# phantomzone-org/fhe-ram

Measured on AMD Instinct MI355X. Metric: encrypted RAM read ops/s + write ops/s at 2^18 entries; achieved HBM GB/s vs peak, higher is better.
Workload: dtype f64

## Files before the change

fhe-ram_amd/csrc/launch.hpp:

```cpp
#pragma once
#include "ctx.hpp"

namespace {

template <typename F>
void with_evk(const fheram_ctx* c, F&& f) {
    if (c->s_evk == 5) f(std::integral_constant<int, 5>{});
    else f(std::integral_constant<int, 4>{});
}
template <typename F>
void with_evk_wide(fheram_ctx* c, bool wide, F&& f) {
    if (wide) c->wide_unsynced = true;
    with_evk(c, [&](auto sk) { if (wide) f(sk, std::true_type{}); else f(sk, std::false_type{}); });
}
bool capturing(const fheram_ctx* c) { return c->use_graph && !c->profile; }

constexpr int LIMB_SPLIT_MAX = 64;
constexpr int EW_SLICES = 8;
int pick_nco(const fheram_ctx* c, int gx, int gy, bool one_wg = false) {
    if (c->nco != 0) return c->nco;
    if (one_wg) return 2;
    return ((long)gx * gy * 2 <= c->cus) ? 1 : 2;
}
void launch_prepare(fheram_ctx* c, const int32_t* in, double* out, int npoly, int64_t gal = 0) {
    ProfScope ps(c, "prepare", npoly);
    const int ginv = gal == 0 ? 0 : galois_inv_mod(galois_mod(gal));
    hipLaunchKernelGGL(k_prepare, dim3((npoly + 1) / 2), dim3(T), LDS_PREPARE_BYTES, c->cur, in, out, c->d_tw, c->ninv, ginv, npoly);
}
double* big_of(const fheram_ctx* c) { return c->cur == c->stream2 ? c->d_big2 : c->d_big; }
bool use_limb_split(const fheram_ctx* c, int gx, int gy, int sk) {
    return c->limb_split && (long)gx * gy <= LIMB_SPLIT_MAX && (long)gx * gy * 2 * sk <= c->cus;
}
bool use_fine_split(const fheram_ctx* c, int gx, int gy, int wgs) {
    return c->limb_split && c->fine_split && (long)gx * gy * wgs <= c->cus && (long)gx * gy * wgs * N * 8 <= (long)LIMB_SPLIT_MAX * BIG_STRIDE * 8;
}
void launch_ep(fheram_ctx* c, GlweRef a, GlweRef res, const double* ggsw, int gx, int gy) {
    if (gx <= 0 || gy <= 0) return;
    ProfScope ps(c, "ext_product", (uint64_t)gx * gy);
    if (use_fine_split(c, gx, gy, 2 * 4 * 2 * 3)) {
        hipLaunchKernelGGL((k_ext_product_fine<3, 4>), dim3(gx, gy, 2 * 4 * 2 * 3), dim3(T), LDS_BYTES, c->cur, a, ggsw, c->d_tw, big_of(c));
        hipLaunchKernelGGL((k_ext_product_fine_norm<3, 4>), dim3(gx, gy, 2 * (N / 256)), dim3(256), 0, c->cur, res, big_of(c));
        return;
    }
    if (use_limb_split(c, gx, gy, 4)) {
        hipLaunchKernelGGL((k_ext_product<3, 4, 1, 1>), dim3(gx, gy, 8), dim3(T), LDS_BYTES, c->cur, a, res, ggsw, c->d_tw, big_of(c));
        hipLaunchKernelGGL((k_ext_product<3, 4, 1, 2>), dim3(gx, gy, 2), dim3(T), 0, c->cur, a, res, ggsw, c->d_tw, big_of(c));
        return;
    }
    if (pick_nco(c, gx, gy) == 1) hipLaunchKernelGGL((k_ext_product<3, 4, 1>), dim3(gx, gy, 2), dim3(T), LDS_BYTES, c->cur, a, res, ggsw, c->d_tw, big_of(c));
    else {
        ProfScope pf(c, "ext_product_fused", (uint64_t)gx * gy);
        hipLaunchKernelGGL((k_ext_product<3, 4, 2>), dim3(gx, gy, 1), dim3(T), LDS_BYTES, c->cur, a, res, ggsw, c->d_tw, big_of(c));
    }
}
template <int MODE, int SX, int SK, int SO>
void launch_ks(fheram_ctx* c, const KsArgs& ka, int gx, int gy) {
    if (gx <= 0 || gy <= 0) return;
    ProfScope ps(c, "keyswitch", (uint64_t)gx * gy);
    if (use_fine_split(c, gx, gy, 2 * SK * SX)) {
        KsArgs kb = ka;
        kb.big = big_of(c);
        hipLaunchKernelGGL((k_keyswitch_fine<MODE, SX, SK>), dim3(gx, gy, 2 * SK * SX), dim3(T), LDS_BYTES, c->cur, kb);
        hipLaunchKernelGGL((k_keyswitch_norm<MODE, SX, SK, SO, SX>), dim3(gx, gy, 2 * (N / 256)), dim3(256), 0, c->cur, kb);
        return;
    }
    if (use_limb_split(c, gx, gy, SK)) {
        KsArgs kb = ka;
        kb.big = big_of(c);
        hipLaunchKernelGGL((k_keyswitch<MODE, SX, SK, SO, 1, 1>), dim3(gx, gy, 2 * SK), dim3(T), LDS_BYTES, c->cur, kb);
        hipLaunchKernelGGL((k_keyswitch_norm<MODE, SX, SK, SO>), dim3(gx, gy, 2 * (N / 256)), dim3(256), 0, c->cur, kb);
        return;
    }
    constexpr bool FUSABLE = (SX == 3) && (MODE != KS_PAIR);
    if constexpr (MODE == KS_PAIR && SX == 3 && SO == 3) {
        if (c->pair_z) {
            hipLaunchKernelGGL((k_pair_z<SK>), dim3(gx, gy, 2), dim3(T), LDS_BYTES, c->cur, ka);
            return;
        }
    }
    if (!FUSABLE || pick_nco(c, gx, gy) == 1) {
        hipLaunchKernelGGL((k_keyswitch<MODE, SX, SK, SO, 1>), dim3(gx, gy, 2), dim3(T), LDS_BYTES, c->cur, ka);
    } else if constexpr (FUSABLE) {
        ProfScope pf(c, "keyswitch_fused", (uint64_t)gx * gy);
        hipLaunchKernelGGL((k_keyswitch<MODE, SX, SK, SO, 2>), dim3(gx, gy, 1), dim3(T), LDS_BYTES, c->cur, ka);
    }
}
void launch_copy(fheram_ctx* c, GlweRef src, GlweRef dst, int gx, int gy) {
    if (gx <= 0 || gy <= 0) return;
    ProfScope ps(c, "elementwise", (uint64_t)gx * gy);
    hipLaunchKernelGGL((k_copy<3>), dim3(gx, gy, EW_SLICES), dim3(256), 0, c->cur, src, dst);
}
KsArgs ks_args(fheram_ctx* c, GlweRef a, GlweRef b, GlweRef out, const double* key, int64_t gal, int t = 0, int rot_mul = 0, int rot_base = 0) {
    KsArgs ka;
    ka.a = a; ka.b = b; ka.out = out; ka.key = key; ka.tw = c->d_tw;
    ka.g = galois_mod(gal); ka.ginv = galois_inv_mod(ka.g); ka.t = t; ka.rot_mul = rot_mul; ka.rot_base = rot_base; ka.big = c->d_big;
    return ka;
}
const double* trace_key(fheram_ctx* c, int i) { return c->d_atk + (size_t)i * c->atk; }
template <int MODE>
void launch_ks_tr(fheram_ctx* c, const KsArgs& ka, int gx, int gy) {
    with_evk(c, [&](auto sk) { launch_ks<MODE, 3, decltype(sk)::value, 3>(c, ka, gx, gy); });
}
bool same(const GlweRef& a, const GlweRef& b) { return a.p == b.p; }

template <typename F>
void run_chain(fheram_ctx* c, int n, GlweRef src, GlweRef dst, GlweRef tmp, int gx, int gy, F&& step) {
    if (n <= 0) { if (!same(src, dst)) launch_copy(c, src, dst, gx, gy); return; }
    if (same(src, dst) && (n % 2 == 1)) {
        run_chain(c, n, src, tmp, dst, gx, gy, step);
        launch_copy(c, tmp, dst, gx, gy);
        return;
    }
    GlweRef cur = src;
    for (int i = 0; i < n; i++) {
        GlweRef out = ((n - 1 - i) % 2 == 0) ? dst : tmp;
        step(i, cur, out);
        cur = out;
    }
}
enum class ChainForm { Tail, Mid, Chain, Steps };
struct ChainPlan {
    ChainForm form;
    int split;
};
struct ChainQuery {
    bool ep;
    int n, gx, gy;
    bool rotated = false;
    bool one_wg = false;
    bool handoff = true;
};
ChainPlan chain_form(const fheram_ctx* c, const ChainQuery& q) {
    const long batch = (long)q.gx * q.gy;
    const int sk = q.ep ? 4 : c->s_evk;
    const bool len = q.n >= 2 && q.n <= CHAIN_MAX;
    const bool handoff = q.handoff && len && c->limb_split &&
                         c->cus >= TAIL_GROUPS * 32 &&
                         !capturing(c);
    if (handoff && !q.ep && !q.rotated && c->tail && c->fine_split && batch <= TAIL_GROUPS &&
        c->cur == c->stream &&
        2 * sk * 3 <= 32)
        return {ChainForm::Tail, 0};
    if (handoff && c->mid && batch > TAIL_GROUPS) {
        if (batch <= 16) return {ChainForm::Mid, 1};
        if (!q.ep && c->mid >= 2) {
            if (batch <= 8 * (32 / (2 * sk))) return {ChainForm::Mid, 2};
            if (batch <= 8 * (32 / sk)) return {ChainForm::Mid, 3};
        }
    }
    if (len && c->chain && pick_nco(c, q.gx, q.gy, q.one_wg) == 2 && !use_limb_split(c, q.gx, q.gy, sk) &&
        !use_fine_split(c, q.gx, q.gy, q.ep ? 2 * 4 * 2 * 3 : 2 * sk * 3))
        return {ChainForm::Chain, 0};
    return {ChainForm::Steps, 0};
}
bool chain_bufs(int n, GlweRef src, GlweRef dst, GlweRef tmp, GlweRef (&b)[2]) {
    if (n % 2 == 1) { if (same(src, dst)) return false; b[0] = dst; b[1] = tmp; }
    else { b[0] = tmp; b[1] = dst; }
    return !same(b[0], src);
}
ChainPlan plan_chain(const fheram_ctx* c, ChainQuery q, GlweRef src, GlweRef dst, GlweRef tmp, GlweRef (&b)[2], bool& fits) {
    fits = chain_bufs(q.n, src, dst, tmp, b);
    ChainPlan p = chain_form(c, q);
    if ((p.form == ChainForm::Tail && !(fits && !same(b[1], src))) || (p.form == ChainForm::Mid && !fits)) {
        q.handoff = false;
        p = chain_form(c, q);
    }
    return p;
}
void mid_rearm(fheram_ctx* c) {
    if (!c->mid && c->mid_saved && ++c->mid_off_ops >= 256) { c->mid = c->mid_saved; c->mid_saved = 0; c->mid_bad_windows = 0; c->mid_off_ops = 0; }
}
template <bool EP>
void fill_mid(fheram_ctx* c, MidArgs& ma, GlweRef src, GlweRef dst, int n, int gx, int gy) {
    const int side = c->cur == c->stream2 ? 1 : 0;
    ma.src = src; ma.dst = dst; ma.tw = c->d_tw; ma.big = c->d_mid_big[side]; ma.sync = c->d_mid_sync[side]; ma.y = c->d_mid_y[side];
    if (++c->mid_seq == 0) ++c->mid_seq;
    c->mid_launches++;
    c->mid_window_cts += (uint64_t)(gx * gy);
    if (!c->mid_test && c->mid_launches - c->mid_launch_mark >= 64) {
        const unsigned fb = __atomic_load_n(c->h_mid_fb, __ATOMIC_RELAXED) + __atomic_load_n(c->h_mid_fb + 16, __ATOMIC_RELAXED);
        const unsigned redone = fb - c->mid_fb_mark;
        const bool bad = (uint64_t)redone * 4u > c->mid_window_cts;
        c->mid_bad_windows = bad ? c->mid_bad_windows + 1 : 0;
        if (c->mid && c->mid_bad_windows >= 2) { c->mid_saved = c->mid; c->mid = 0; c->mid_disabled_count++; }
        c->mid_fb_mark = fb;
        c->mid_launch_mark = c->mid_launches;
        c->mid_window_cts = 0;
    }
    ma.seq = c->mid_seq; ma.n = n; ma.n_ct = gx * gy; ma.gx = gx; ma.rot_mul = 0; ma.rot_base = 0;
    ma.give_up_at = c->mid_test ? n - 2 : -1;
}
template <int SK, int RS, int LPM>
void launch_k_mid_trace(fheram_ctx* c, const MidArgs& ma) {
    constexpr int members = RS * 2 * SK / LPM;
    hipLaunchKernelGGL((k_chain_mid<false, SK, RS, LPM>), dim3(8 * (32 / members) * members), dim3(T), LDS_BYTES, c->cur, ma);
}
void launch_mid_trace(fheram_ctx* c, GlweRef src, const GlweRef (&b)[2], int start, int n, int gx, int gy, int rot_mul, int rot_base, int split) {
    ProfScope ps(c, "keyswitch", (uint64_t)gx * gy, n);
    ProfScope pm(c, "keyswitch_mid_launch", (uint64_t)gx * gy * n, 1);
    MidArgs ma;
    fill_mid<false>(c, ma, src, b[(n - 1) & 1], n, gx, gy);
    ma.rot_mul = rot_mul; ma.rot_base = rot_base;
    KsChainArgs ca;
    ca.base = ks_args(c, src, src, b[0], trace_key(c, start), c->gal[start], 0, rot_mul, rot_base);
    ca.buf[0] = b[0]; ca.buf[1] = b[1]; ca.n = n;
    ca.done = ma.sync; ca.done_seq = ma.seq; ca.host_count = c->h_mid_fb + (c->cur == c->stream2 ? 16 : 0);
    for (int i = 0; i < n; i++) { ma.opnd[i] = ca.key[i] = trace_key(c, start + i); ma.ginv[i] = ca.ginv[i] = galois_inv_mod(galois_mod(c->gal[start + i])); }
    with_evk(c, [&](auto sk) {
        constexpr int SK = decltype(sk)::value;
        if (split == 1) launch_k_mid_trace<SK, 3, 2>(c, ma); else if (split == 2) launch_k_mid_trace<SK, 1, 1>(c, ma); else launch_k_mid_trace<SK, 1, 2>(c, ma);
        hipLaunchKernelGGL((k_keyswitch_chain<3, SK, 3>), dim3(gx, gy, 1), dim3(T), LDS_BYTES, c->cur, ca);
    });
}
void launch_mid_ep(fheram_ctx* c, GlweRef src, const GlweRef (&b)[2], const double* prep, int d, int gx, int gy) {
    ProfScope ps(c, "ext_product", (uint64_t)gx * gy, d);
    ProfScope pm(c, "ext_product_mid_launch", (uint64_t)gx * gy * d, 1);
    MidArgs ma;
    fill_mid<true>(c, ma, src, b[(d - 1) & 1], d, gx, gy);
    EpChainArgs ca;
    ca.src = src; ca.buf[0] = b[0]; ca.buf[1] = b[1]; ca.tw = c->d_tw; ca.n = d;
    ca.done = ma.sync; ca.done_seq = ma.seq; ca.host_count = c->h_mid_fb + (c->cur == c->stream2 ? 16 : 0);
    for (int i = 0; i < d; i++) { ma.opnd[i] = ca.ggsw[i] = prep + (size_t)i * fheram_ctx::GGSW; ma.ginv[i] = 1; }
    hipLaunchKernelGGL((k_chain_mid<true, 4, 3, 2>), dim3(8 * 2 * 12), dim3(T), LDS_BYTES, c->cur, ma);
    hipLaunchKernelGGL((k_ext_product_chain<3, 4>), dim3(gx, gy, 1), dim3(T), LDS_BYTES, c->cur, ca);
}
void launch_ep_chain(fheram_ctx* c, GlweRef src, const GlweRef (&b)[2], const double* prep, int d, int gx, int gy) {
    ProfScope ps(c, "ext_product", (uint64_t)gx * gy, d);
    ProfScope pf(c, "ext_product_fused", (uint64_t)gx * gy, d);
    EpChainArgs ca;
    ca.src = src; ca.buf[0] = b[0]; ca.buf[1] = b[1]; ca.tw = c->d_tw; ca.n = d;
    for (int i = 0; i < d; i++) ca.ggsw[i] = prep + (size_t)i * fheram_ctx::GGSW;
    if (d >= 2) hipLaunchKernelGGL((k_ext_product_chain_r<4>), dim3(gx, gy, 1), dim3(T), LDS_BYTES, c->cur, ca);
    else hipLaunchKernelGGL((k_ext_product_chain<3, 4>), dim3(gx, gy, 1), dim3(T), LDS_BYTES, c->cur, ca);
}
void ep_chain(fheram_ctx* c, GlweRef src, GlweRef dst, GlweRef tmp, const double* prep, int d, int gx, int gy) {
    if (gx <= 0 || gy <= 0) return;
    GlweRef b[2];
    bool fits;
    switch (plan_chain(c, ChainQuery{true, d, gx, gy}, src, dst, tmp, b, fits).form) {
    case ChainForm::Mid: launch_mid_ep(c, src, b, prep, d, gx, gy); return;
    case ChainForm::Chain:
        if (!fits && !chain_bufs(d, src, tmp, dst, b)) break;
        launch_ep_chain(c, src, b, prep, d, gx, gy);
        if (!fits) launch_copy(c, tmp, dst, gx, gy);
        return;
    default: break;
    }
    run_chain(c, d, src, dst, tmp, gx, gy, [&](int i, GlweRef in, GlweRef out) { launch_ep(c, in, out, prep + (size_t)i * fheram_ctx::GGSW, gx, gy); });
}
void launch_trace_chain(fheram_ctx* c, GlweRef src, const GlweRef (&b)[2], int start, int n, int gx, int gy, int rot_mul, int rot_base) {
    ProfScope ps(c, "keyswitch", (uint64_t)gx * gy, n);
    ProfScope pf(c, "keyswitch_fused", (uint64_t)gx * gy, n);
    ProfScope pl(c, "keyswitch_chain_launch", (uint64_t)gx * gy * n, 1);
    KsChainArgs ca;
    ca.base = ks_args(c, src, src, b[0], trace_key(c, start), c->gal[start], 0, rot_mul, rot_base);
    ca.buf[0] = b[0]; ca.buf[1] = b[1]; ca.n = n;
    for (int i = 0; i < n; i++) { ca.key[i] = trace_key(c, start + i); ca.ginv[i] = galois_inv_mod(galois_mod(c->gal[start + i])); }
    const int yf = n >= 2 ? c->chain_y : 0;
    with_evk_wide(c, yf && c->wide, [&](auto sk, auto w) {
        constexpr int SK = decltype(sk)::value;
        if (!yf) hipLaunchKernelGGL((k_keyswitch_chain<3, SK, 3>), dim3(gx, gy, 1), dim3(T), LDS_BYTES, c->cur, ca);
        else if constexpr (decltype(w)::value) hipLaunchKernelGGL((k_keyswitch_chain_w<3, SK, 3, 3>), dim3(gx, gy, 1), dim3(T), LDS_BYTES, c->cur, ca);
        else hipLaunchKernelGGL((k_keyswitch_chain<3, SK, 3, 3>), dim3(gx, gy, 1), dim3(T), LDS_BYTES, c->cur, ca);
    });
}
struct OpndTable { int ws = 0; long stride = 0; unsigned src_map = 0; };
constexpr unsigned SRC_MAP_IDENTITY = 0x76543210u;
bool use_row_fuse(const fheram_ctx* c, int d, int n_tr, int gx, int gy, bool one_wg = false) {
    return c->fuse && c->chain_y == 3 && !capturing(c) &&
           chain_form(c, ChainQuery{true, d, gx, gy, false, one_wg}).form == ChainForm::Chain &&
           chain_form(c, ChainQuery{false, n_tr, gx, gy, false, one_wg}).form == ChainForm::Chain;
}
RowChainTableArgs with_table(const RowChainArgs& ra, const OpndTable& t) {
    RowChainTableArgs rt;
    static_cast<RowChainArgs&>(rt) = ra;
    rt.opnd_stride = t.stride; rt.ws = t.ws; rt.src_map = t.src_map;
    return rt;
}
void fill_row_chain(fheram_ctx* c, RowChainArgs& ra, const double* prep, int d, int start, int n_tr) {
    ra.ep.tw = c->d_tw; ra.ep.n = d;
    for (int i = 0; i < d; i++) ra.ep.ggsw[i] = prep + (size_t)i * fheram_ctx::GGSW;
    ra.ks.n = n_tr;
    for (int i = 0; i < n_tr; i++) { ra.ks.key[i] = trace_key(c, start + i); ra.ks.ginv[i] = galois_inv_mod(galois_mod(c->gal[start + i])); }
}
void launch_read_chain(fheram_ctx* c, GlweRef src, const GlweRef* ep_store, GlweRef dst, const double* prep, int d, int n_tr, int gx, int gy, const OpndTable& t) {
    ProfScope ps(c, "read_chain_launch", (uint64_t)gx * gy, 1);
    RowChainArgs ra;
    fill_row_chain(c, ra, prep, d, 0, n_tr);
    ra.ep.src = src;
    ra.ep.buf[0] = ra.ep.buf[1] = ep_store ? *ep_store : dst;
    ra.store_ep = ep_store ? 1 : 0;
    ra.ks.base = ks_args(c, dst, dst, dst, trace_key(c, 0), c->gal[0]);
    ra.ks.buf[0] = ra.ks.buf[1] = dst;
    ra.hi = dst; ra.trhi = dst;
    if (t.ws > 0) {
        c->wide_unsynced = true;
        with_evk(c, [&](auto sk) {
            constexpr int SK = decltype(sk)::value;
            hipLaunchKernelGGL((k_read_chain_t<SK, 4>), dim3(gx, gy, 1), dim3(T), LDS_BYTES, c->cur, with_table(ra, t));
        });
        return;
    }
    with_evk_wide(c, c->wide, [&](auto sk, auto w) {
        constexpr int SK = decltype(sk)::value;
        if constexpr (decltype(w)::value) hipLaunchKernelGGL((k_read_chain_w<SK, 4>), dim3(gx, gy, 1), dim3(T), LDS_BYTES, c->cur, ra);
        else hipLaunchKernelGGL((k_read_chain<SK, 4>), dim3(gx, gy, 1), dim3(T), LDS_BYTES, c->cur, ra);
    });
}
void launch_write_chain(fheram_ctx* c, GlweRef src, int rot_mul, int rot_base, GlweRef data, GlweRef trhi, const double* prep, int d, int n_tr, int gx, int gy, const OpndTable& t) {
    ProfScope ps(c, "write_chain_launch", (uint64_t)gx * gy, 1);
    RowChainArgs ra;
    fill_row_chain(c, ra, prep, d, 0, n_tr);
    ra.ks.base = ks_args(c, src, src, data, trace_key(c, 0), c->gal[0], 0, rot_mul, rot_base);
    ra.ks.buf[0] = ra.ks.buf[1] = data;
    ra.hi = data; ra.trhi = trhi;
    ra.ep.src = data; ra.ep.buf[0] = ra.ep.buf[1] = data;
    c->wide_unsynced = true;
    with_evk(c, [&](auto sk) {
        constexpr int SK = decltype(sk)::value;
        if (t.ws > 0) hipLaunchKernelGGL((k_write_chain_t<SK, 4>), dim3(gx, gy, 1), dim3(T), LDS_BYTES, c->cur, with_table(ra, t));
        else hipLaunchKernelGGL((k_write_chain<SK, 4>), dim3(gx, gy, 1), dim3(T), LDS_BYTES, c->cur, ra);
    });
}
void launch_trace_tail(fheram_ctx* c, GlweRef src, const GlweRef (&b)[2], int start, int n, int gx, int gy,
                       const double* prep = nullptr, int d = 0, GlweRef ep_out = GlweRef{nullptr, 0, 0}, bool store_ep = false, const OpndTable& t = {}) {
    ProfScope ps(c, "keyswitch", (uint64_t)gx * gy, n);
    ProfScope pt(c, "keyswitch_tail_launch", (uint64_t)gx * gy * n, 1);
    TailArgs ta;
    ta.src = src; ta.buf[0] = b[0]; ta.buf[1] = b[1]; ta.tw = c->d_tw; ta.big = big_of(c); ta.sync = c->d_tail_sync;
    ta.n_ep = prep ? d : 0; ta.ep_out = ep_out;
    for (int i = 0; i < TAIL_EP_MAX; i++) ta.ggsw[i] = (prep && i < d) ? prep + (size_t)i * fheram_ctx::GGSW : nullptr;
    if (++c->tail_seq == 0) ++c->tail_seq;
    c->tail_launches++;
    if (c->tail_test != 1 && c->tail_launches - c->tail_launch_mark >= 64) {
        const unsigned fb = *(volatile unsigned*)c->h_tail_fb;
        if (fb - c->tail_fb_mark > 16) c->tail = 0;
        c->tail_fb_mark = fb;
        c->tail_launch_mark = c->tail_launches;
    }
    ta.seq = c->tail_seq; ta.n = n; ta.n_ct = gx * gy; ta.gx = gx; ta.xoff = c->tail_xoff; ta.give_up_at = c->tail_test ? ta.n_ep + n - 2 : -1;
    KsChainArgs ca;
    ca.base = ks_args(c, src, src, b[0], trace_key(c, start), c->gal[start], 0, 0, 0);
    ca.buf[0] = b[0]; ca.buf[1] = b[1]; ca.n = n;
    ca.pred = c->d_tail_sync + TAIL_GROUPS * 32; ca.pred_seq = ta.seq; ca.host_count = c->h_tail_fb;
    for (int i = 0; i < n; i++) { ta.key[i] = ca.key[i] = trace_key(c, start + i); ta.ginv[i] = ca.ginv[i] = galois_inv_mod(galois_mod(c->gal[start + i])); }
    RowChainArgs ra;
    if (ta.n_ep) {
        fill_row_chain(c, ra, prep, d, start, n);
        ra.ep.src = src; ra.ep.buf[0] = ra.ep.buf[1] = ep_out; ra.store_ep = store_ep ? 1 : 0;
        ra.ks.base = ks_args(c, b[(n - 1) & 1], b[(n - 1) & 1], b[(n - 1) & 1], trace_key(c, start), c->gal[start]);
        ra.ks.buf[0] = ra.ks.buf[1] = b[(n - 1) & 1];
        ra.hi = ra.trhi = b[(n - 1) & 1];
        ra.ks.pred = ca.pred; ra.ks.pred_seq = ca.pred_seq; ra.ks.host_count = ca.host_count;
    }
    with_evk(c, [&](auto sk) {
        constexpr int SK = decltype(sk)::value;
        const dim3 groups(TAIL_GROUPS * 2 * SK * 3);
        if (t.ws > 0 && ta.n_ep) {
            TailTableArgs tt;
            static_cast<TailArgs&>(tt) = ta;
            tt.opnd_stride = t.stride; tt.ws = t.ws;
            hipLaunchKernelGGL((k_trace_tail_t<3, SK, 3>), groups, dim3(T), LDS_BYTES, c->cur, tt);
            c->wide_unsynced = true;
            hipLaunchKernelGGL((k_read_chain_t<SK, 4>), dim3(gx, gy, 1), dim3(T), LDS_BYTES, c->cur, with_table(ra, OpndTable{t.ws, t.stride, SRC_MAP_IDENTITY}));
            return;
        }
        hipLaunchKernelGGL((k_trace_tail<3, SK, 3>), groups, dim3(T), LDS_BYTES, c->cur, ta);
        if (ta.n_ep) hipLaunchKernelGGL((k_read_chain<SK, 4>), dim3(gx, gy, 1), dim3(T), LDS_BYTES, c->cur, ra);
        else hipLaunchKernelGGL((k_keyswitch_chain<3, SK, 3>), dim3(gx, gy, 1), dim3(T), LDS_BYTES, c->cur, ca);
    });
}
void trace_steps(fheram_ctx* c, GlweRef src, GlweRef dst, GlweRef tmp, int start, int end, int gx, int gy, int rot_mul = 0, int rot_base = 0) {
    if (gx <= 0 || gy <= 0) return;
    const int n = end - start;
    GlweRef b[2];
    bool fits;
    const ChainPlan p = plan_chain(c, ChainQuery{false, n, gx, gy, rot_mul != 0 || rot_base != 0}, src, dst, tmp, b, fits);
    switch (p.form) {
    case ChainForm::Tail: launch_trace_tail(c, src, b, start, n, gx, gy); return;
    case ChainForm::Mid: launch_mid_trace(c, src, b, start, n, gx, gy, rot_mul, rot_base, p.split); return;
    case ChainForm::Chain:
        if (!fits && !chain_bufs(n, src, tmp, dst, b)) break;
        launch_trace_chain(c, src, b, start, n, gx, gy, rot_mul, rot_base);
        if (!fits) launch_copy(c, tmp, dst, gx, gy);
        return;
    case ChainForm::Steps: break;
    }
    run_chain(c, n, src, dst, tmp, gx, gy, [&](int i, GlweRef in, GlweRef out) {
        KsArgs ka = ks_args(c, in, in, out, trace_key(c, start + i), c->gal[start + i], 0, i == 0 ? rot_mul : 0, i == 0 ? rot_base : 0);
        launch_ks_tr<KS_TRACE>(c, ka, gx, gy);
    });
}
int32_t* pack_levels(fheram_ctx* c, int32_t* src, int32_t* A, int32_t* B, long sy, long sx, size_t count, int gy,
                     int n_alone, int first_pair, bool keep_alone = false, int32_t* P0 = nullptr, int32_t* P1 = nullptr) {
    const int k = ilog2_ceil(count);
    int32_t* cur = src;
    auto other = [&](int32_t* x) { return x == A ? B : A; };
    if (n_alone > 0 && count > 0) {
        int32_t* b0 = other(src);
        int32_t* b1 = other(b0);
        if (b1 == src && P0 && P0 != src && chain_form(c, ChainQuery{false, n_alone, (int)count, gy}).form == ChainForm::Tail) b1 = P0;
        cur = keep_alone ? A : ((n_alone - 1) & 1) ? b1 : b0;
        trace_steps(c, ref(src, sy, sx), ref(cur, sy, sx), ref(cur == b0 ? b1 : b0, sy, sx), 0, n_alone, (int)count, gy);
    }
    size_t live = count;
    for (int m = 0; m < k; m++) {
        const int i = first_pair + m;
        const long h = (long)1 << (k - 1 - m);
        int32_t* nxt = (keep_alone && P0) ? (cur == P0 ? P1 : P0) : other(cur);
        const long n_pair = std::max<long>(0, std::min<long>(h, (long)live - h));
        const long n_alone_here = std::min<long>(h, (long)live) - n_pair;
        if (n_pair > 0) {
            KsArgs ka = ks_args(c, ref(cur, sy, sx), ref(cur + h * sx, sy, sx), ref(nxt, sy, sx), trace_key(c, i), c->gal[i], N >> (i + 1));
            launch_ks_tr<KS_PAIR>(c, ka, (int)n_pair, gy);
        }
        if (n_alone_here > 0) {
            KsArgs ka = ks_args(c, ref(cur + n_pair * sx, sy, sx), ref(cur, sy, sx), ref(nxt + n_pair * sx, sy, sx), trace_key(c, i), c->gal[i]);
            launch_ks_tr<KS_TRACE>(c, ka, (int)n_alone_here, gy);
        }
        live = std::min<size_t>(live, (size_t)h);
        cur = nxt;
    }
    return cur;
}
int coord_first_digit(const fheram_ctx* c, int ci) { int s = 0; for (int i = 0; i < ci; i++) s += (int)c->base2d[i].size(); return s; }
double* digits_of(const fheram_ctx* c, double* table, int ci) { return table + (size_t)coord_first_digit(c, ci) * fheram_ctx::GGSW; }
void coordinate_prepare(fheram_ctx* c, const fheram_addr* addr, int ci, double* table) {
    const int d = (int)c->base2d[ci].size();
    launch_prepare(c, addr->d_ggsw + (size_t)coord_first_digit(c, ci) * fheram_ctx::GGSW, digits_of(c, table, ci), d * (int)(fheram_ctx::GGSW / N));
}
void coordinate_prepare_all(fheram_ctx* c, const fheram_addr* addr, double* table) {
    launch_prepare(c, addr->d_ggsw, table, c->n_digits * (int)(fheram_ctx::GGSW / N));
}
void ggsw_inverse(fheram_ctx* c, const int32_t* in, int32_t* tmp, int d) {
    const long g4 = (long)fheram_ctx::GLWE4;
    int32_t* inp = const_cast<int32_t*>(in);
    KsArgs ka = ks_args(c, ref(inp, (long)fheram_ctx::GGSW, 2 * g4), ref(inp, 0, 0), ref(tmp, (long)fheram_ctx::GGSW, 2 * g4), c->d_atk_inv, -1);
    launch_ks<KS_AUTO, 4, 5, 4>(c, ka, fheram_ctx::DNUM_CT, d);
    KsArgs kt = ks_args(c, ref(tmp, (long)fheram_ctx::GGSW, 2 * g4), ref(tmp, 0, 0), ref(tmp + g4, (long)fheram_ctx::GGSW, 2 * g4), c->d_tsk, 1);
    launch_ks<KS_TENSOR, 4, 5, 4>(c, kt, fheram_ctx::DNUM_CT, d);
}
void coordinate_prepare_inv(fheram_ctx* c, const fheram_addr* addr, int ci, int32_t* tmp, double* prep) {
    const int d = (int)c->base2d[ci].size();
    ggsw_inverse(c, addr->d_ggsw + (size_t)coord_first_digit(c, ci) * fheram_ctx::GGSW, tmp, d);
    launch_prepare(c, tmp, prep, d * (int)(fheram_ctx::GGSW / N));
}

void precompute_inverse(fheram_ctx* c, const fheram_addr* addr, int ci, bool fork, unsigned gate_seq = 0) {
    if (fork && c->wdone_pending) {
        hipStreamWaitEvent(c->stream2, c->ev_wdone, 0);
        c->wdone_pending = false;
    }
    if (fork && gate_seq) {
        if (c->opstart_valid) { hipStreamWaitEvent(c->stream2, c->ev_opstart, 0); c->opstart_valid = false; }
        hipLaunchKernelGGL(k_tail_gate, dim3(1), dim3(64), 0, c->stream2, c->d_tail_sync + TAIL_GROUPS * 32 + 2, gate_seq);
    } else if (fork) {
        hipEventRecord(c->ev_fork, c->stream);
        hipStreamWaitEvent(c->stream2, c->ev_fork, 0);
    }
    hipStream_t keep = c->cur;
    c->cur = c->stream2;
    coordinate_prepare_inv(c, addr, ci, c->d_ggsw_inv + (size_t)coord_first_digit(c, ci) * fheram_ctx::GGSW, digits_of(c, c->d_prep_inv, ci));
    hipEventRecord(c->ev_inv[ci], c->stream2);
    c->cur = keep;
    c->inv_id[ci] = addr->id;
    c->inv_pending[ci] = true;
}
void wait_inverse(fheram_ctx* c, hipStream_t s, int ci) { if (!capturing(c)) hipStreamWaitEvent(s, c->ev_inv[ci], 0); }

}
```

fhe-ram_amd/csrc/path.hpp:

```cpp
#pragma once
#include "launch.hpp"

namespace {

struct Opnds {
    fheram_ctx* c;
    RamState* st;
    const fheram_addr* const* addrs;
    int n, ws;
    double *tab, *tab_inv;
    long stride;
    unsigned src_map;
    bool bank;
    int member(int k) const { return (int)((src_map >> (4 * k)) & 15u); }
    int Y() const { return n * ws; }
    double* prep(int k, int ci) const { return digits_of(c, tab + k * stride, ci); }
    double* inv(int k, int ci) const { return digits_of(c, tab_inv + k * stride, ci); }
    GlweRef slice(GlweRef r, int k) const { r.p += (long)k * ws * r.sy; return r; }
    GlweRef rows(GlweRef r, int k) const { return slice(r, member(k)); }
    OpndTable table() const { return n == 1 ? OpndTable{} : OpndTable{ws, stride, src_map}; }
    bool row_fuse(int d, int n_tr, int gx) const { return use_row_fuse(c, d, n_tr, gx, Y(), bank); }
};
Opnds one_addr(fheram_ctx* c, const fheram_addr* const* a, int ws, RamState* st) { return Opnds{c, st, a, 1, ws, c->d_prep, c->d_prep_inv, 0, 0, false}; }
Opnds one_addr(fheram_ctx* c, const fheram_addr* const* a) { return one_addr(c, a, c->ws, &c->ram); }
Opnds table_opnds(fheram_ctx* c, RamState* st, const fheram_addr* const* addrs, int n, int ws, double* tab, double* tab_inv, unsigned src_map, bool bank) {
    return Opnds{c, st, addrs, n, ws, tab, tab_inv, (long)c->n_digits * (long)fheram_ctx::GGSW, src_map, bank};
}

struct RamView {
    int32_t *rows, *A, *B, *C, *D;
    int32_t *part, *tmp, *tmp2, *res, *tree, *w, *trtop;
};
RamView ctx_view(const fheram_ctx* c) {
    return RamView{c->d_data, c->d_scrA, c->d_scrB, c->d_scrC, c->d_scrD, c->d_part, c->d_tmp, c->d_tmp2, c->d_res, c->d_tree, c->d_w, c->d_trtop};
}

void read_local_done(const fheram_ctx* c, RamState* st, bool prepare_write) {
    if (c->n2 == 2) st->memo_alone = (prepare_write && c->memo) ? LOGN - ilog2_ceil(c->rows_glob) : 0;
}
void read_top_done(fheram_ctx* c, RamState* st, bool prepare_write) {
    st->memo_top = prepare_write && c->memo;
    st->res_in_trtop = st->memo_top;
    c->prep1_ready = false;
}
void write_done(fheram_ctx* c, RamState* st) { st->memo_top = false; st->memo_alone = 0; c->side_begun = false; c->tree_rotate_pending = false; }

template <typename F>
int run_op(fheram_ctx* c, const fheram_addr* addr, int which, F&& enqueue) {
    if (!c->use_graph || c->profile) return enqueue();
    fheram_addr* a = const_cast<fheram_addr*>(addr);
    const unsigned sig = 1u | (c->ram.memo_top ? 2u : 0u) | ((unsigned)c->ram.memo_alone << 2) | (c->side_begun ? 64u : 0u) |
                         (c->inv_id[0] == addr->id ? 128u : 0u) | (c->inv_id[1] == addr->id ? 256u : 0u);
    if (a->graph[which] && a->graph_sig[which] != sig) { hipGraphExecDestroy(a->graph[which]); a->graph[which] = nullptr; }
    if (!a->graph[which]) {
        hipGraph_t g = nullptr;
        HIPCHK(c, hipStreamBeginCapture(c->stream, hipStreamCaptureModeThreadLocal));
        const int rc = enqueue();
        const hipError_t e = hipStreamEndCapture(c->stream, &g);
        if (rc != FHERAM_OK || e != hipSuccess) {
            if (g) hipGraphDestroy(g);
            return rc != FHERAM_OK ? rc : fail(c, FHERAM_ERR_DEVICE, std::string("hipStreamEndCapture: ") + hipGetErrorString(e));
        }
        const hipError_t e2 = hipGraphInstantiate(&a->graph[which], g, nullptr, nullptr, 0);
        hipGraphDestroy(g);
        if (e2 != hipSuccess) { a->graph[which] = nullptr; return fail(c, FHERAM_ERR_DEVICE, std::string("hipGraphInstantiate: ") + hipGetErrorString(e2)); }
        a->graph_sig[which] = sig;
    }
    HIPCHK(c, hipGraphLaunch(a->graph[which], c->stream));
    if (which == 2) write_done(c, &c->ram);
    else { read_local_done(c, &c->ram, which == 1); read_top_done(c, &c->ram, which == 1); }
    return FHERAM_OK;
}

int check_common(fheram_ctx* c, const fheram_addr* addr) {
    if (!c) return FHERAM_ERR_INVALID_ARG;
    mid_rearm(c);
    if (!addr || addr->ctx != c) return fail(c, FHERAM_ERR_INVALID_ARG, "address does not belong to this context (layout mismatch, ram.rs:404)");
    if (addr->empty) return fail(c, FHERAM_ERR_INVALID_ARG, "empty address: fheram_address_alloc without fheram_address_derive");
    if (!c->ram.initialized) return fail(c, FHERAM_ERR_UNINITIALIZED, "unitialized memory: self.data.len()=0");
    if (!c->keys_loaded) return fail(c, FHERAM_ERR_KEYS, "evaluation keys not loaded");
    return FHERAM_OK;
}

int read_local(const Opnds& o, const RamView& a, bool prepare_write, GlweRef* packed_out, bool to_part) {
    fheram_ctx* c = o.c;
    const int n = o.n, ws = o.ws, Y = o.Y(), R = (int)c->rows;
    c->wide = !prepare_write || n > 1;
    if (n == 1 && prepare_write && c->pre_inv == 1 && !capturing(c) && (c->wide_unsynced || c->derive_unsynced)) {
        hipEventRecord(c->ev_opstart, c->stream);
        c->opstart_valid = true;
    }
    const long G = (long)fheram_ctx::GLWE;
    const long sy = (long)c->rows * G;
    GlweRef data = ref(a.rows, sy, G), A = ref(a.A, sy, G), B = ref(a.B, sy, G);
    GlweRef part = ref(a.part, G, 0);
    const bool all = (c->n_shards == 1 && c->n2 == 2);
    for (int k = 0; k < n; k++)
        if (all) coordinate_prepare_all(c, o.addrs[k], o.tab + k * o.stride); else coordinate_prepare(c, o.addrs[k], 0, o.tab + k * o.stride);
    c->prep1_ready = all;
    read_local_done(c, o.st, prepare_write);
    const int d0 = (int)c->base2d[0].size();
    if (c->n2 == 1) {
        GlweRef row0 = ref(a.rows, sy, 0);
        for (int k = 0; k < n; k++)
            if (prepare_write) ep_chain(c, o.rows(row0, k), o.rows(row0, k), o.slice(ref(a.A, sy, 0), k), o.prep(k, 0), d0, 1, ws);
            else ep_chain(c, o.rows(row0, k), o.slice(part, k), o.slice(ref(a.tmp, G, 0), k), o.prep(k, 0), d0, 1, ws);
        *packed_out = prepare_write ? row0 : part;
        if (prepare_write && to_part) launch_copy(c, row0, part, 1, Y);
        return FHERAM_OK;
    }
    const int L0 = LOGN - ilog2_ceil(c->rows_glob);
    const bool keep = o.st->memo_alone > 0;
    int32_t* packed;
    if (o.row_fuse(d0, L0, R) && !(prepare_write && (d0 & 1))) {
        launch_read_chain(c, data, prepare_write ? &data : nullptr, A, o.prep(0, 0), d0, L0, R, Y, o.table());
        packed = pack_levels(c, a.A, a.A, a.B, sy, G, (size_t)R, Y, 0, L0, keep, a.C, a.D);
    } else {
        for (int k = 0; k < n; k++)
            if (prepare_write) ep_chain(c, o.rows(data, k), o.rows(data, k), o.slice(A, k), o.prep(k, 0), d0, R, ws);
            else ep_chain(c, o.rows(data, k), o.slice(A, k), o.slice(B, k), o.prep(k, 0), d0, R, ws);
        packed = pack_levels(c, prepare_write ? a.rows : a.A, a.A, a.B, sy, G, (size_t)R, Y, L0, L0, keep, a.C, a.D);
    }
    *packed_out = ref(packed, sy, 0);
    if (to_part) launch_copy(c, *packed_out, part, 1, Y);
    return FHERAM_OK;
}
int read_top(const Opnds& o, const RamView& a, bool prepare_write, int32_t* gathered, GlweRef pk) {
    fheram_ctx* c = o.c;
    const int n = o.n, ws = o.ws, Y = o.Y();
    c->wide = !prepare_write || n > 1;
    const long G = (long)fheram_ctx::GLWE;
    GlweRef tmp = ref(a.tmp, G, 0);
    GlweRef last = pk;
    const int d1 = c->n2 == 2 ? (int)c->base2d[1].size() : 0;
    auto tail_top = [&] { return chain_form(c, ChainQuery{false, LOGN, 1, Y}).form == ChainForm::Tail; };
    const bool fuse_ep = c->n2 == 2 && c->tail_ep && d1 >= 2 && d1 <= TAIL_EP_MAX && tail_top();
    GlweRef ep_out = ref(prepare_write ? a.tree : a.tmp2, G, 0);
    auto products1 = [&] { for (int k = 0; k < n; k++) ep_chain(c, o.slice(pk, k), o.slice(ep_out, k), o.slice(tmp, k), o.prep(k, 1), d1, 1, ws); };
    if (c->n2 == 2) {
        if (gathered) {
            const int kG = ilog2_ceil((size_t)c->n_shards);
            int32_t* a0 = c->d_gat[1];
            int32_t* a1 = c->d_gat[2];
            int32_t* packed = pack_levels(c, gathered, a0, a1, G, (long)ws * G, (size_t)c->n_shards, ws, 0, LOGN - kG);
            pk = ref(packed, G, 0);
        }
        if (!c->prep1_ready) coordinate_prepare(c, o.addrs[0], 1, o.tab);
        if (!fuse_ep) products1();
        last = ep_out;
    }
    const bool pre = n == 1 && prepare_write && c->pre_inv && (long)c->rows * Y <= c->cus;
    const bool gated = pre && c->pre_inv == 1 && !capturing(c) && tail_top();
    if (pre && !gated)
        for (int ci = c->n2 - 1; ci >= 0; ci--) precompute_inverse(c, o.addrs[0], ci, ci == c->n2 - 1);
    read_top_done(c, o.st, prepare_write);
    const GlweRef res = ref(o.st->memo_top ? a.trtop : a.res, G, 0);
    const uint64_t tl0 = c->tail_launches;
    GlweRef tb[2];
    if (fuse_ep && chain_bufs(LOGN, last, res, tmp, tb))
        launch_trace_tail(c, pk, tb, 0, LOGN, 1, Y, o.prep(0, 1), d1, ep_out, prepare_write, o.table());
    else {
        if (fuse_ep) products1();
        trace_steps(c, last, res, tmp, 0, LOGN, 1, Y);
    }
    if (gated && !c->opstart_valid && (c->wide_unsynced || c->derive_unsynced)) {
        hipEventRecord(c->ev_opstart, c->stream);
        c->opstart_valid = true;
    }
    if (gated) {
        const unsigned seq = c->tail_launches != tl0 ? c->tail_seq : 0;
        for (int ci = c->n2 - 1; ci >= 0; ci--) precompute_inverse(c, o.addrs[0], ci, ci == c->n2 - 1, seq);
    }
    return FHERAM_OK;
}
int read_impl(const Opnds& o, const RamView& a, bool prepare_write) {
    fheram_ctx* c = o.c;
    GlweRef packed;
    int rc = read_local(o, a, prepare_write, &packed, false);
    if (rc != FHERAM_OK) return rc;
    rc = read_top(o, a, prepare_write, nullptr, packed);
    if (o.n == 1 && prepare_write && c->inv_id[0] == o.addrs[0]->id && capturing(c))
        for (int ci = 0; ci < c->n2; ci++) hipStreamWaitEvent(c->stream, c->ev_inv[ci], 0);
    if (rc == FHERAM_OK && prepare_write) o.st->state = true;
    return rc;
}

void reads_free(ReadBufs& L) {
    void* bufs[] = {L.A, L.B, L.C, L.res, L.tmp, L.tmp2, L.prep};
    for (void* p : bufs) if (p) hipFree(p);
    if (L.h_res) hipHostFree(L.h_res);
    L = ReadBufs{};
}
bool third_arena_needed(const fheram_ctx* c, int n_ct) {
    return c->n2 == 2 && chain_form(c, ChainQuery{false, LOGN - ilog2_ceil(c->rows_glob), (int)c->rows, n_ct}).form == ChainForm::Tail;
}
int reads_reserve(fheram_ctx* c, ReadBufs& L, int n, int ws) {
    const bool work = n > 1, third = work && third_arena_needed(c, n * ws);
    if (n <= L.cap && (!work || L.A) && (!third || L.C)) return FHERAM_OK;
    if (n < L.cap) n = L.cap;
    const bool had_work = L.A != nullptr, had_third = L.C != nullptr;
    if (L.cap) { HIPCHK(c, hipStreamSynchronize(c->stream)); reads_free(L); }
    const size_t G = fheram_ctx::GLWE, nct = (size_t)n * ws, nrow = nct * c->rows;
    hipError_t e = hipSuccess;
    auto dev = [&](auto** p, size_t bytes) { if (e == hipSuccess) e = hipMalloc((void**)p, bytes); };
    dev(&L.res, nct * G * sizeof(int32_t));
    if (work || had_work) {
        dev(&L.A, nrow * G * sizeof(int32_t));
        dev(&L.B, nrow * G * sizeof(int32_t));
        if (third || had_third) dev(&L.C, nrow * G * sizeof(int32_t));
        dev(&L.tmp, nct * G * sizeof(int32_t));
        dev(&L.tmp2, nct * G * sizeof(int32_t));
        dev(&L.prep, (size_t)n * c->n_digits * fheram_ctx::GGSW * sizeof(double));
    }
    if (e == hipSuccess) e = hipHostMalloc((void**)&L.h_res, (nct * G + 1) * sizeof(int64_t), hipHostMallocMapped);
    if (e == hipSuccess) e = hipHostGetDevicePointer((void**)&L.d_h_res, L.h_res, 0);
    if (e != hipSuccess) {
        reads_free(L);
        (void)hipGetLastError();
        return fail(c, FHERAM_ERR_DEVICE, std::string("read buffers for ") + std::to_string(n) + " addresses: " + hipGetErrorString(e));
    }
    L.cap = n;
    return FHERAM_OK;
}
RamView reads_view(const fheram_ctx* c, const ReadBufs& L) { return RamView{c->d_data, L.A, L.B, L.C, nullptr, L.tmp2, L.tmp, L.tmp2, L.res, nullptr, nullptr, nullptr}; }

struct ResRun { const int32_t* src; size_t n; };
int result_export(fheram_ctx* c, const ResRun* runs, int n_runs, int64_t* h, int64_t* d_h, int64_t* out) {
    size_t n = 0;
    for (int i = 0; i < n_runs; i++) {
        const int n4 = (int)(runs[i].n / 4);
        hipLaunchKernelGGL(k_export_i64, dim3((n4 + 255) / 256), dim3(256), 0, c->stream, runs[i].src, reinterpret_cast<long long*>(d_h + n), n4,
                           reinterpret_cast<const long long*>(c->d_tw + N));
        n += runs[i].n;
    }
    HIPCHK(c, hipStreamSynchronize(c->stream));
    HIPCHK(c, hipGetLastError());
    c->wide_unsynced = c->derive_unsynced = false;
    double m;
    std::memcpy(&m, h + n, 8);
    if (c->monitor && m > MON_LIMIT) __atomic_store_n(c->h_ro_flag, 1u, __ATOMIC_RELAXED);
    const int rc = check_precision(c);
    if (rc == FHERAM_OK && out) std::memcpy(out, h, n * sizeof(int64_t));
    return rc;
}

int reads_export(fheram_ctx* c, const ReadBufs& L, size_t first, size_t n_ct, int64_t* out) {
    const ResRun run{L.res + first * fheram_ctx::GLWE, n_ct * fheram_ctx::GLWE};
    return result_export(c, &run, 1, L.h_res, L.d_h_res, out);
}
template <typename F>
int read_many(fheram_ctx* c, ReadBufs& L, RamState* st, const fheram_addr* const* addrs, int n, int ws, unsigned src_map, bool bank, int64_t* out, F&& kept) {
    int rc = reads_reserve(c, L, n, ws);
    if (rc != FHERAM_OK) return rc;
    const Opnds o = table_opnds(c, st, addrs, n, ws, L.prep, nullptr, src_map, bank);
    rc = read_impl(o, reads_view(c, L), false);
    if (rc != FHERAM_OK) return rc;
    kept(o);
    HIPCHK(c, hipGetLastError());
    return out ? reads_export(c, L, 0, (size_t)n * ws, out) : FHERAM_OK;
}

int write_top(const Opnds& o, const RamView& v) {
    fheram_ctx* c = o.c;
    c->wide = true;
    const long G = (long)fheram_ctx::GLWE;
    const long sy = (long)c->rows * G;
    const int n = o.n, ws = o.ws, Y = o.Y();
    GlweRef wref = ref(v.w, G, 0), tmp = ref(v.tmp, G, 0), tmp2 = ref(v.tmp2, G, 0), tree = ref(v.tree, G, 0);
    GlweRef top = (c->n2 != 1) ? tree : ref(v.rows, sy, 0);
    GlweRef tr = tmp;
    if (o.st->memo_top) tr = ref(v.trtop, G, 0);
    else trace_steps(c, top, tmp, tmp2, 0, LOGN, 1, Y);
    {
        ProfScope ps(c, "elementwise", Y);
        hipLaunchKernelGGL((k_sub_add_norm<3>), dim3(1, Y, EW_SLICES), dim3(256), 0, c->cur, top, tr, wref, top);
    }
    o.st->memo_top = false;
    if (c->n2 == 2) {
        if (n == 1 && c->inv_id[1] == o.addrs[0]->id) wait_inverse(c, c->stream, 1);
        else {
            if (n == 1 && c->inv_pending[1]) wait_inverse(c, c->stream, 1);
            for (int k = 0; k < n; k++) coordinate_prepare_inv(c, o.addrs[k], 1, c->d_ggsw_tmp, o.inv(k, 1));
        }
        if (n == 1) { c->inv_pending[1] = false; c->inv_id[1] = 0; }
        for (int k = 0; k < n; k++)
            ep_chain(c, o.slice(tree, k), o.slice(ref(v.part, G, 0), k), o.slice(tmp, k), o.inv(k, 1), (int)c->base2d[1].size(), 1, ws);
        c->tree_rotate_pending = true;
    }
    return FHERAM_OK;
}
void write_side_begin(const Opnds& o, const RamView& v) {
    fheram_ctx* c = o.c;
    c->wide = true;
    const long G = (long)fheram_ctx::GLWE;
    const long sy = (long)c->rows * G;
    hipEventRecord(c->ev_fork, c->stream);
    hipStreamWaitEvent(c->stream2, c->ev_fork, 0);
    c->cur = c->stream2;
    if (c->n2 == 2) {
        const int kept = o.st->memo_alone;
        c->trhi_in_C = kept > 0 && (LOGN - kept) % 2 == 1;
        if (kept > 0) trace_steps(c, ref(v.A, sy, G), ref(c->trhi_in_C ? v.C : v.A, sy, G), ref(c->trhi_in_C ? v.A : v.C, sy, G), kept, LOGN, (int)c->rows, o.Y());
        else trace_steps(c, ref(v.rows, sy, G), ref(v.A, sy, G), ref(v.C, sy, G), 0, LOGN, (int)c->rows, o.Y());
        o.st->memo_alone = 0;
    }
    if (o.n == 1 && c->inv_id[0] == o.addrs[0]->id) wait_inverse(c, c->stream2, 0);
    else for (int k = 0; k < o.n; k++) coordinate_prepare_inv(c, o.addrs[k], 0, c->d_ggsw_tmp2, o.inv(k, 0));
    if (o.n == 1) { c->inv_id[0] = 0; c->inv_pending[0] = false; }
    hipEventRecord(c->ev_join, c->stream2);
    c->cur = c->stream;
    c->side_begun = true;
}
void write_side_abort(fheram_ctx* c) {
    if (!c->side_begun) return;
    hipStreamWaitEvent(c->stream, c->ev_join, 0);
    c->side_begun = false;
}
int write_rows(const Opnds& o, const RamView& v) {
    fheram_ctx* c = o.c;
    c->wide = true;
    const long G = (long)fheram_ctx::GLWE;
    const long sy = (long)c->rows * G;
    const int n = o.n, ws = o.ws, Y = o.Y(), R = (int)c->rows;
    GlweRef data = ref(v.rows, sy, G), A = ref(v.A, sy, G), B = ref(v.B, sy, G), D = ref(v.D, sy, G);
    GlweRef trhi = ref(c->trhi_in_C ? v.C : v.A, sy, G), part = ref(v.part, G, 0);
    const int d0 = (int)c->base2d[0].size();
    const bool fuse = c->n2 == 2 && o.row_fuse(d0, LOGN, R);
    if (fuse) {
        hipStreamWaitEvent(c->stream, c->ev_join, 0);
        launch_write_chain(c, part, c->n_shards, c->shard, data, trhi, o.inv(0, 0), d0, LOGN, R, Y, o.table());
    } else if (c->n2 == 2)
        trace_steps(c, part, B, D, 0, LOGN, R, Y, c->n_shards, c->shard);
    if (c->tree_rotate_pending) {
        ProfScope ps(c, "elementwise", Y);
        hipLaunchKernelGGL((k_rotate<3>), dim3(1, Y, EW_SLICES), dim3(256), 0, c->cur, part, ref(v.tree, G, 0), -(int)c->rows_glob);
    }
    if (!fuse) {
        hipStreamWaitEvent(c->stream, c->ev_join, 0);
        if (c->n2 == 2) {
            ProfScope ps(c, "elementwise", (uint64_t)R * Y);
            hipLaunchKernelGGL((k_sub_add_norm<3>), dim3(R, Y, EW_SLICES), dim3(256), 0, c->cur, data, trhi, B, data);
        }
        for (int k = 0; k < n; k++) ep_chain(c, o.slice(data, k), o.slice(data, k), o.slice(A, k), o.inv(k, 0), d0, R, ws);
    }
    if (n == 1 && !capturing(c)) { hipEventRecord(c->ev_wdone, c->stream); c->wdone_pending = true; }
    write_done(c, o.st);
    o.st->state = false;
    return FHERAM_OK;
}

}
```

Measured before the change: 1304.

## Batch inverse-GGSW precompute across coordinates with side-stream workgroup budget

Replaces the per-coordinate inverse precompute loop with one batched call that runs the automorphism and tensor keyswitches and the prepare over all digits at once on the side stream. Keyswitch split heuristics now take a workgroup budget, so the side-stream work sizes its split or fusion choice to a reserved share of CUs (TAIL_GROUPS times the CUs left per XCD) instead of the whole device. The aim is fewer launches and less contention with the concurrent tail kernels. The trade-off is that all coordinates' inverses now complete together, so events for earlier coordinates fire later.

```diff
diff --git a/fhe-ram_amd/csrc/launch.hpp b/fhe-ram_amd/csrc/launch.hpp
--- a/fhe-ram_amd/csrc/launch.hpp
+++ b/fhe-ram_amd/csrc/launch.hpp
@@ -17,10 +17,11 @@
 
 constexpr int LIMB_SPLIT_MAX = 64;
 constexpr int EW_SLICES = 8;
-int pick_nco(const fheram_ctx* c, int gx, int gy, bool one_wg = false) {
+int wg_budget(const fheram_ctx* c, int budget) { return budget > 0 ? budget : c->cus; }
+int pick_nco(const fheram_ctx* c, int gx, int gy, bool one_wg = false, int budget = 0) {
     if (c->nco != 0) return c->nco;
     if (one_wg) return 2;
-    return ((long)gx * gy * 2 <= c->cus) ? 1 : 2;
+    return ((long)gx * gy * 2 <= wg_budget(c, budget)) ? 1 : 2;
 }
 void launch_prepare(fheram_ctx* c, const int32_t* in, double* out, int npoly, int64_t gal = 0) {
     ProfScope ps(c, "prepare", npoly);
@@ -28,11 +29,11 @@
     hipLaunchKernelGGL(k_prepare, dim3((npoly + 1) / 2), dim3(T), LDS_PREPARE_BYTES, c->cur, in, out, c->d_tw, c->ninv, ginv, npoly);
 }
 double* big_of(const fheram_ctx* c) { return c->cur == c->stream2 ? c->d_big2 : c->d_big; }
-bool use_limb_split(const fheram_ctx* c, int gx, int gy, int sk) {
-    return c->limb_split && (long)gx * gy <= LIMB_SPLIT_MAX && (long)gx * gy * 2 * sk <= c->cus;
-}
-bool use_fine_split(const fheram_ctx* c, int gx, int gy, int wgs) {
-    return c->limb_split && c->fine_split && (long)gx * gy * wgs <= c->cus && (long)gx * gy * wgs * N * 8 <= (long)LIMB_SPLIT_MAX * BIG_STRIDE * 8;
+bool use_limb_split(const fheram_ctx* c, int gx, int gy, int sk, int budget = 0) {
+    return c->limb_split && (long)gx * gy <= LIMB_SPLIT_MAX && (long)gx * gy * 2 * sk <= wg_budget(c, budget);
+}
+bool use_fine_split(const fheram_ctx* c, int gx, int gy, int wgs, int budget = 0) {
+    return c->limb_split && c->fine_split && (long)gx * gy * wgs <= wg_budget(c, budget) && (long)gx * gy * wgs * N * 8 <= (long)LIMB_SPLIT_MAX * BIG_STRIDE * 8;
 }
 void launch_ep(fheram_ctx* c, GlweRef a, GlweRef res, const double* ggsw, int gx, int gy) {
     if (gx <= 0 || gy <= 0) return;
@@ -54,17 +55,17 @@
     }
 }
 template <int MODE, int SX, int SK, int SO>
-void launch_ks(fheram_ctx* c, const KsArgs& ka, int gx, int gy) {
+void launch_ks(fheram_ctx* c, const KsArgs& ka, int gx, int gy, int budget = 0) {
     if (gx <= 0 || gy <= 0) return;
     ProfScope ps(c, "keyswitch", (uint64_t)gx * gy);
-    if (use_fine_split(c, gx, gy, 2 * SK * SX)) {
+    if (use_fine_split(c, gx, gy, 2 * SK * SX, budget)) {
         KsArgs kb = ka;
         kb.big = big_of(c);
         hipLaunchKernelGGL((k_keyswitch_fine<MODE, SX, SK>), dim3(gx, gy, 2 * SK * SX), dim3(T), LDS_BYTES, c->cur, kb);
         hipLaunchKernelGGL((k_keyswitch_norm<MODE, SX, SK, SO, SX>), dim3(gx, gy, 2 * (N / 256)), dim3(256), 0, c->cur, kb);
         return;
     }
-    if (use_limb_split(c, gx, gy, SK)) {
+    if (use_limb_split(c, gx, gy, SK, budget)) {
         KsArgs kb = ka;
         kb.big = big_of(c);
         hipLaunchKernelGGL((k_keyswitch<MODE, SX, SK, SO, 1, 1>), dim3(gx, gy, 2 * SK), dim3(T), LDS_BYTES, c->cur, kb);
@@ -78,7 +79,7 @@
             return;
         }
     }
-    if (!FUSABLE || pick_nco(c, gx, gy) == 1) {
+    if (!FUSABLE || pick_nco(c, gx, gy, false, budget) == 1) {
         hipLaunchKernelGGL((k_keyswitch<MODE, SX, SK, SO, 1>), dim3(gx, gy, 2), dim3(T), LDS_BYTES, c->cur, ka);
     } else if constexpr (FUSABLE) {
         ProfScope pf(c, "keyswitch_fused", (uint64_t)gx * gy);
@@ -432,13 +433,13 @@
 void coordinate_prepare_all(fheram_ctx* c, const fheram_addr* addr, double* table) {
     launch_prepare(c, addr->d_ggsw, table, c->n_digits * (int)(fheram_ctx::GGSW / N));
 }
-void ggsw_inverse(fheram_ctx* c, const int32_t* in, int32_t* tmp, int d) {
+void ggsw_inverse(fheram_ctx* c, const int32_t* in, int32_t* tmp, int d, int budget = 0) {
     const long g4 = (long)fheram_ctx::GLWE4;
     int32_t* inp = const_cast<int32_t*>(in);
     KsArgs ka = ks_args(c, ref(inp, (long)fheram_ctx::GGSW, 2 * g4), ref(inp, 0, 0), ref(tmp, (long)fheram_ctx::GGSW, 2 * g4), c->d_atk_inv, -1);
-    launch_ks<KS_AUTO, 4, 5, 4>(c, ka, fheram_ctx::DNUM_CT, d);
+    launch_ks<KS_AUTO, 4, 5, 4>(c, ka, fheram_ctx::DNUM_CT, d, budget);
     KsArgs kt = ks_args(c, ref(tmp, (long)fheram_ctx::GGSW, 2 * g4), ref(tmp, 0, 0), ref(tmp + g4, (long)fheram_ctx::GGSW, 2 * g4), c->d_tsk, 1);
-    launch_ks<KS_TENSOR, 4, 5, 4>(c, kt, fheram_ctx::DNUM_CT, d);
+    launch_ks<KS_TENSOR, 4, 5, 4>(c, kt, fheram_ctx::DNUM_CT, d, budget);
 }
 void coordinate_prepare_inv(fheram_ctx* c, const fheram_addr* addr, int ci, int32_t* tmp, double* prep) {
     const int d = (int)c->base2d[ci].size();
@@ -446,25 +447,30 @@
     launch_prepare(c, tmp, prep, d * (int)(fheram_ctx::GGSW / N));
 }
 
-void precompute_inverse(fheram_ctx* c, const fheram_addr* addr, int ci, bool fork, unsigned gate_seq = 0) {
-    if (fork && c->wdone_pending) {
+constexpr int SIDE_WG_PER_XCD = 32 - 2 * 4 * 3;
+constexpr int SIDE_WG_BUDGET = TAIL_GROUPS * SIDE_WG_PER_XCD;
+void precompute_inverse_all(fheram_ctx* c, const fheram_addr* addr, unsigned gate_seq = 0) {
+    if (c->wdone_pending) {
         hipStreamWaitEvent(c->stream2, c->ev_wdone, 0);
         c->wdone_pending = false;
     }
-    if (fork && gate_seq) {
+    if (gate_seq) {
         if (c->opstart_valid) { hipStreamWaitEvent(c->stream2, c->ev_opstart, 0); c->opstart_valid = false; }
         hipLaunchKernelGGL(k_tail_gate, dim3(1), dim3(64), 0, c->stream2, c->d_tail_sync + TAIL_GROUPS * 32 + 2, gate_seq);
-    } else if (fork) {
+    } else {
         hipEventRecord(c->ev_fork, c->stream);
         hipStreamWaitEvent(c->stream2, c->ev_fork, 0);
     }
     hipStream_t keep = c->cur;
     c->cur = c->stream2;
-    coordinate_prepare_inv(c, addr, ci, c->d_ggsw_inv + (size_t)coord_first_digit(c, ci) * fheram_ctx::GGSW, digits_of(c, c->d_prep_inv, ci));
-    hipEventRecord(c->ev_inv[ci], c->stream2);
+    ggsw_inverse(c, addr->d_ggsw, c->d_ggsw_inv, c->n_digits, SIDE_WG_BUDGET);
+    launch_prepare(c, c->d_ggsw_inv, c->d_prep_inv, c->n_digits * (int)(fheram_ctx::GGSW / N));
     c->cur = keep;
-    c->inv_id[ci] = addr->id;
-    c->inv_pending[ci] = true;
+    for (int ci = c->n2 - 1; ci >= 0; ci--) {
+        hipEventRecord(c->ev_inv[ci], c->stream2);
+        c->inv_id[ci] = addr->id;
+        c->inv_pending[ci] = true;
+    }
 }
 void wait_inverse(fheram_ctx* c, hipStream_t s, int ci) { if (!capturing(c)) hipStreamWaitEvent(s, c->ev_inv[ci], 0); }
 
diff --git a/fhe-ram_amd/csrc/path.hpp b/fhe-ram_amd/csrc/path.hpp
--- a/fhe-ram_amd/csrc/path.hpp
+++ b/fhe-ram_amd/csrc/path.hpp
@@ -151,8 +151,7 @@
     }
     const bool pre = n == 1 && prepare_write && c->pre_inv && (long)c->rows * Y <= c->cus;
     const bool gated = pre && c->pre_inv == 1 && !capturing(c) && tail_top();
-    if (pre && !gated)
-        for (int ci = c->n2 - 1; ci >= 0; ci--) precompute_inverse(c, o.addrs[0], ci, ci == c->n2 - 1);
+    if (pre && !gated) precompute_inverse_all(c, o.addrs[0]);
     read_top_done(c, o.st, prepare_write);
     const GlweRef res = ref(o.st->memo_top ? a.trtop : a.res, G, 0);
     const uint64_t tl0 = c->tail_launches;
@@ -169,7 +168,7 @@
     }
     if (gated) {
         const unsigned seq = c->tail_launches != tl0 ? c->tail_seq : 0;
-        for (int ci = c->n2 - 1; ci >= 0; ci--) precompute_inverse(c, o.addrs[0], ci, ci == c->n2 - 1, seq);
+        precompute_inverse_all(c, o.addrs[0], seq);
     }
     return FHERAM_OK;
 }
```

Result: no change. 1315, median of 6 (+0.9%).
